# ViTAE-Transformer/SAMRS

Hardware: AMD Instinct MI355X
Metric: images/sec (1024^2, vit_h, 32 boxes/img) SAM box->mask (higher is better)
Workload: dtype f16

## Files before the change

### samrs_amd/csrc/decoder_kernels.hip

```cpp
#include "common.h"
#include "kernels.h"
#include "postprocess_value.h"

namespace {

constexpr float TWO_PI = 6.283185307179586f;

__device__ __forceinline__ float pe_channel(const float* __restrict__ gauss, float cx01, float cy01, int ch, int half) {
    const int f = ch < half ? ch : ch - half;
    const float vx = 2.0f * cx01 - 1.0f, vy = 2.0f * cy01 - 1.0f;
    const float a = TWO_PI * (vx * gauss[f] + vy * gauss[half + f]);
    return ch < half ? sinf(a) : cosf(a);
}

__global__ void prompt_tokens_kernel(PromptParams p, float* __restrict__ tokens, float* __restrict__ tokens2, int T, int C) {
    const int j = blockIdx.x, b = blockIdx.y, ch = threadIdx.x;
    const int half = C / 2;
    const bool has_pts = p.point_coords != nullptr;
    const bool has_box = p.boxes != nullptr;
    const int npt = has_pts ? p.n_points + (has_box ? 0 : 1) : 0;
    float v;
    if (j == 0) {
        v = p.iou_token[ch];
    } else if (j < 5) {
// ... 235 lines not shown
            }
#pragma unroll
            for (int t = 0; t < T2I_TG; ++t) {
                float sc = 0.f;
#pragma unroll
                for (int c = 0; c < 8; ++c) sc += q[t][c] * kf[c];
                sc += __builtin_bit_cast(float, __builtin_amdgcn_update_dpp(0, __builtin_bit_cast(int, sc), 0xB1, 0xF, 0xF, true));
                sc = valid ? sc : T2I_NEG;
                const float mn = fmaxf(m[t], sc);
                const float corr = __builtin_amdgcn_exp2f(m[t] - mn);
                const float pj = valid ? __builtin_amdgcn_exp2f(sc - mn) : 0.f;
                l[t] = l[t] * corr + pj;
#pragma unroll
                for (int c = 0; c < 8; ++c) acc[t][c] = acc[t][c] * corr + pj * vf[c];
                m[t] = mn;
            }
        }
#pragma unroll
        for (int u = 0; u < U; ++u) { kk[u] = kn[u]; vv[u] = vn[u]; }
    }
#undef T2I_LOAD
#pragma unroll
    for (int off = 16; off <= 32; off <<= 1) {
#pragma unroll
        for (int t = 0; t < T2I_TG; ++t) {
            const float mo = __shfl_xor(m[t], off, 64), lo = __shfl_xor(l[t], off, 64);
            const float mn = fmaxf(m[t], mo);
            const float fs = __builtin_amdgcn_exp2f(m[t] - mn), fo = __builtin_amdgcn_exp2f(mo - mn);
            l[t] = l[t] * fs + lo * fo;
#pragma unroll
            for (int c = 0; c < 8; ++c) acc[t][c] = acc[t][c] * fs + __shfl_xor(acc[t][c], off, 64) * fo;
            m[t] = mn;
        }
    }
    if (lane < 16) {
#pragma unroll
        for (int t = 0; t < T2I_TG; ++t) {
            float* r = sm[wave][t][ch];
            r[0] = m[t]; r[1] = l[t];
#pragma unroll
            for (int c = 0; c < 8; ++c) r[2 + c] = acc[t][c];
        }
    }
    __syncthreads();
    if (threadIdx.x < T2I_TG * 16) {
        const int t = threadIdx.x >> 4, c16 = threadIdx.x & 15;
        float mm = sm[0][t][c16][0];
#pragma unroll
        for (int w = 1; w < 4; ++w) mm = fmaxf(mm, sm[w][t][c16][0]);
        float ll = 0.f, a[8] = {0.f, 0.f, 0.f, 0.f, 0.f, 0.f, 0.f, 0.f};
#pragma unroll
        for (int w = 0; w < 4; ++w) {
            const float f = __builtin_amdgcn_exp2f(sm[w][t][c16][0] - mm);
            ll += sm[w][t][c16][1] * f;
#pragma unroll
            for (int c = 0; c < 8; ++c) a[c] += sm[w][t][c16][2 + c] * f;
        }
        float* r = part + ((((size_t)b * gridDim.z + blockIdx.z) * gridDim.x + split) * (T2I_TG * 16) + threadIdx.x) * T2I_REC;
        r[0] = mm; r[1] = ll;
#pragma unroll
        for (int c = 0; c < 8; ++c) r[2 + c] = a[c];
    }
}

__global__ __launch_bounds__(T2I_TG * 16) void t2i_merge_kernel(const float* __restrict__ part, float* __restrict__ o,
                                                                int splits, int T, int Ci) {
    const int b = blockIdx.x, tg = blockIdx.y;
    const int t = tg * T2I_TG + (threadIdx.x >> 4), ch = threadIdx.x & 15;
    if (t >= T) return;
    const float* base = part + (((size_t)b * gridDim.y + tg) * splits * (T2I_TG * 16) + threadIdx.x) * T2I_REC;
    const size_t sstride = (size_t)(T2I_TG * 16) * T2I_REC;
    float mm = T2I_NEG;
    for (int s = 0; s < splits; ++s) mm = fmaxf(mm, base[s * sstride]);
    float ll = 0.f, a[8] = {0.f, 0.f, 0.f, 0.f, 0.f, 0.f, 0.f, 0.f};
    for (int s = 0; s < splits; ++s) {
        const float* r = base + s * sstride;
        const float f = __builtin_amdgcn_exp2f(r[0] - mm);
        ll += r[1] * f;
#pragma unroll
        for (int c = 0; c < 8; ++c) a[c] += r[2 + c] * f;
    }
    const float inv = 1.0f / ll;
    float* orow = o + ((size_t)b * T + t) * Ci + ch * 8;
#pragma unroll
    for (int c = 0; c < 8; ++c) orow[c] = a[c] * inv;
}

constexpr int I2T_HS = 20;
template <int PREC>
__global__ __launch_bounds__(256) void i2t_attention_kernel(const uint16_t* __restrict__ qi, int ld, long bstride,
                                                            const float* __restrict__ kt, const float* __restrict__ vt,
                                                            uint16_t* __restrict__ out, int T, int tokens, int Ci) {
    constexpr int HD = 16;
    extern __shared__ float sm[];
    const int heads = Ci / HD;
    const int RS = heads * I2T_HS;
    float* sk = sm;
    float* sv = sm + T * RS;
    const int b = blockIdx.y;
    for (int i = threadIdx.x; i < T * Ci; i += 256) {
        const int j = i / Ci, c = i % Ci;
        sk[j * RS + (c / HD) * I2T_HS + c % HD] = kt[(size_t)b * T * Ci + i];
        sv[j * RS + (c / HD) * I2T_HS + c % HD] = vt[(size_t)b * T * Ci + i];
    }
    __syncthreads();
    const int tok = blockIdx.x * (256 / heads) + threadIdx.x / heads;
    const int h = threadIdx.x % heads;
    if (tok >= tokens) return;
    const uint16_t* qrow = qi + ((size_t)b * bstride + tok) * ld + h * HD;
    const uint4 q0 = *reinterpret_cast<const uint4*>(qrow);
    const uint4 q1 = *reinterpret_cast<const uint4*>(qrow + 8);
    const uint32_t qw[8] = {q0.x, q0.y, q0.z, q0.w, q1.x, q1.y, q1.z, q1.w};
    float qf[HD];
#pragma unroll
    for (int c = 0; c < 8; ++c) {
        qf[2 * c] = ET<PREC>::to_float((uint16_t)(qw[c] & 0xffffu)) * 0.25f;
        qf[2 * c + 1] = ET<PREC>::to_float((uint16_t)(qw[c] >> 16)) * 0.25f;
    }
    float m = -INFINITY, l = 0.f, acc[HD];
#pragma unroll
    for (int c = 0; c < HD; ++c) acc[c] = 0.f;
    for (int j = 0; j < T; ++j) {
        float kr[HD], vr[HD];
#pragma unroll
        for (int c4 = 0; c4 < HD / 4; ++c4) {
            const float4 k4 = *reinterpret_cast<const float4*>(sk + j * RS + h * I2T_HS + 4 * c4);
            const float4 v4 = *reinterpret_cast<const float4*>(sv + j * RS + h * I2T_HS + 4 * c4);
            kr[4 * c4] = k4.x; kr[4 * c4 + 1] = k4.y; kr[4 * c4 + 2] = k4.z; kr[4 * c4 + 3] = k4.w;
            vr[4 * c4] = v4.x; vr[4 * c4 + 1] = v4.y; vr[4 * c4 + 2] = v4.z; vr[4 * c4 + 3] = v4.w;
        }
        float s = 0.f;
#pragma unroll
        for (int c = 0; c < HD; ++c) s += qf[c] * kr[c];
        const float mn = fmaxf(m, s);
        const float corr = __expf(m - mn), pj = __expf(s - mn);
        l = l * corr + pj;
#pragma unroll
        for (int c = 0; c < HD; ++c) acc[c] = acc[c] * corr + pj * vr[c];
        m = mn;
    }
    const float inv = 1.0f / l;
    uint4 o0, o1;
    o0.x = pack2<PREC>(acc[0] * inv, acc[1] * inv);   o0.y = pack2<PREC>(acc[2] * inv, acc[3] * inv);
    o0.z = pack2<PREC>(acc[4] * inv, acc[5] * inv);   o0.w = pack2<PREC>(acc[6] * inv, acc[7] * inv);
    o1.x = pack2<PREC>(acc[8] * inv, acc[9] * inv);   o1.y = pack2<PREC>(acc[10] * inv, acc[11] * inv);
    o1.z = pack2<PREC>(acc[12] * inv, acc[13] * inv); o1.w = pack2<PREC>(acc[14] * inv, acc[15] * inv);
    uint16_t* orow = out + ((size_t)b * tokens + tok) * Ci + h * HD;
    *reinterpret_cast<uint4*>(orow) = o0;
    *reinterpret_cast<uint4*>(orow + 8) = o1;
}

constexpr int I2TF_ROWS = 32;
constexpr int I2TF_AST = 136;

template <int PREC, bool SPLIT>
__global__ __launch_bounds__(256, 2) void i2t_fused_kernel(const uint16_t* __restrict__ qi, int ld, long q_bstride,
                                                        const int* __restrict__ slot_of, const float* __restrict__ kt, const float* __restrict__ vt,
                                                        const uint16_t* __restrict__ w, const uint16_t* __restrict__ w_lo,
                                                        const float* __restrict__ bias,
                                                        const float* __restrict__ resid, long r_bstride,
                                                        const float* __restrict__ gamma, const float* __restrict__ beta, float eps,
                                                        float* __restrict__ outF, uint16_t* __restrict__ outE,
                                                        uint16_t* __restrict__ outE_lo, int T, int tokens, int groups_per_block) {
    constexpr int HD = 16, HEADS = 8, CI = 128, CO = 256, NWV = 4;
    constexpr int KRS = HEADS * I2T_HS;
    extern __shared__ __attribute__((aligned(16))) unsigned char smraw[];
    float* sk = reinterpret_cast<float*>(smraw);
    float* sv = sk + T * KRS;
    float* sp = sv + T * KRS;
    float* ex = sp + 3 * CO;
    uint16_t* At = reinterpret_cast<uint16_t*>(ex + 2 * NWV * I2TF_ROWS);
    uint16_t* Al = At + I2TF_ROWS * I2TF_AST;
    const int tid = threadIdx.x, lane = tid & 63, wave = tid >> 6;
    const int fr = lane & 15, fq = lane >> 4;
    const int b = blockIdx.y;
    for (int i = tid; i < T * CI; i += 256) {
        const int j = i / CI, c = i % CI;
        sk[j * KRS + (c / HD) * I2T_HS + c % HD] = kt[(size_t)b * T * CI + i];
        sv[j * KRS + (c / HD) * I2T_HS + c % HD] = vt[(size_t)b * T * CI + i];
    }
    for (int i = tid; i < CO; i += 256) { sp[i] = bias[i]; sp[CO + i] = gamma[i]; sp[2 * CO + i] = beta[i]; }
    uint4 wf[4][4], wl[SPLIT ? 4 : 1][4];
#pragma unroll
    for (int i = 0; i < 4; ++i)
#pragma unroll
        for (int ks = 0; ks < 4; ++ks) {
            const size_t o = (size_t)(wave * 64 + i * 16 + fr) * CI + ks * 32 + fq * 8;
            wf[i][ks] = *reinterpret_cast<const uint4*>(w + o);
            if constexpr (SPLIT) wl[i][ks] = *reinterpret_cast<const uint4*>(w_lo + o);
        }
    __syncthreads();

    const int tr = tid >> 3, h = tid & 7;
    const int g0 = blockIdx.x * groups_per_block;
    const int ib = slot_of ? slot_of[b] : b;
    const uint16_t* qbase = qi + (size_t)ib * q_bstride * ld + (size_t)tr * ld + h * HD;
    uint4 q0 = make_uint4(0u, 0u, 0u, 0u), q1 = q0;
    if (g0 * I2TF_ROWS < tokens) {
        q0 = *reinterpret_cast<const uint4*>(qbase + (size_t)g0 * I2TF_ROWS * ld);
        q1 = *reinterpret_cast<const uint4*>(qbase + (size_t)g0 * I2TF_ROWS * ld + 8);
    }
    for (int g = g0; g < g0 + groups_per_block; ++g) {
        const int row0 = g * I2TF_ROWS;
        if (row0 >= tokens) break;
        float4 rs[2][4];
#pragma unroll
        for (int mt = 0; mt < 2; ++mt)
#pragma unroll
            for (int i = 0; i < 4; ++i)
                rs[mt][i] = *reinterpret_cast<const float4*>(resid + ((size_t)ib * r_bstride + row0 + mt * 16 + fr) * CO + wave * 64 + i * 16 + 4 * fq);
        {
            const uint32_t qw[8] = {q0.x, q0.y, q0.z, q0.w, q1.x, q1.y, q1.z, q1.w};
            float qf[HD];
#pragma unroll
            for (int c = 0; c < 8; ++c) {
                qf[2 * c] = ET<PREC>::to_float((uint16_t)(qw[c] & 0xffffu)) * 0.25f;
                qf[2 * c + 1] = ET<PREC>::to_float((uint16_t)(qw[c] >> 16)) * 0.25f;
            }
            float m = -INFINITY, l = 0.f, acc[HD];
#pragma unroll
            for (int c = 0; c < HD; ++c) acc[c] = 0.f;
            for (int j = 0; j < T; ++j) {
                float kr[HD], vr[HD];
#pragma unroll
                for (int c4 = 0; c4 < HD / 4; ++c4) {
                    const float4 k4 = *reinterpret_cast<const float4*>(sk + j * KRS + h * I2T_HS + 4 * c4);
                    const float4 v4 = *reinterpret_cast<const float4*>(sv + j * KRS + h * I2T_HS + 4 * c4);
                    kr[4 * c4] = k4.x; kr[4 * c4 + 1] = k4.y; kr[4 * c4 + 2] = k4.z; kr[4 * c4 + 3] = k4.w;
                    vr[4 * c4] = v4.x; vr[4 * c4 + 1] = v4.y; vr[4 * c4 + 2] = v4.z; vr[4 * c4 + 3] = v4.w;
                }
                float sc = 0.f;
#pragma unroll
                for (int c = 0; c < HD; ++c) sc += qf[c] * kr[c];
                const float mn = fmaxf(m, sc);
                const float corr = __expf(m - mn), pj = __expf(sc - mn);
                l = l * corr + pj;
#pragma unroll
                for (int c = 0; c < HD; ++c) acc[c] = acc[c] * corr + pj * vr[c];
                m = mn;
            }
            const float inv = 1.0f / l;
            uint32_t oh[8], ol[8];
#pragma unroll
            for (int c = 0; c < 8; ++c) split2_pack<PREC>(acc[2 * c] * inv, acc[2 * c + 1] * inv, oh[c], ol[c]);
            *reinterpret_cast<uint4*>(At + tr * I2TF_AST + h * HD) = make_uint4(oh[0], oh[1], oh[2], oh[3]);
            *reinterpret_cast<uint4*>(At + tr * I2TF_AST + h * HD + 8) = make_uint4(oh[4], oh[5], oh[6], oh[7]);
            if constexpr (SPLIT) {
                *reinterpret_cast<uint4*>(Al + tr * I2TF_AST + h * HD) = make_uint4(ol[0], ol[1], ol[2], ol[3]);
                *reinterpret_cast<uint4*>(Al + tr * I2TF_AST + h * HD + 8) = make_uint4(ol[4], ol[5], ol[6], ol[7]);
            }
        }
        __syncthreads();
        if (g + 1 < g0 + groups_per_block && (g + 1) * I2TF_ROWS < tokens) {
            q0 = *reinterpret_cast<const uint4*>(qbase + (size_t)(g + 1) * I2TF_ROWS * ld);
            q1 = *reinterpret_cast<const uint4*>(qbase + (size_t)(g + 1) * I2TF_ROWS * ld + 8);
        }
        float v[2][4][4];
        float s1[2];
#pragma unroll
        for (int mt = 0; mt < 2; ++mt) {
            uint4 af[4], al[SPLIT ? 4 : 1];
#pragma unroll
            for (int ks = 0; ks < 4; ++ks) {
                af[ks] = *reinterpret_cast<const uint4*>(At + (mt * 16 + fr) * I2TF_AST + ks * 32 + fq * 8);
                if constexpr (SPLIT) al[ks] = *reinterpret_cast<const uint4*>(Al + (mt * 16 + fr) * I2TF_AST + ks * 32 + fq * 8);
            }
            s1[mt] = 0.f;
#pragma unroll
            for (int i = 0; i < 4; ++i) {
                f32x4_t a = {0.f, 0.f, 0.f, 0.f};
                if constexpr (SPLIT) {
                    f32x4_t c = {0.f, 0.f, 0.f, 0.f};
#pragma unroll
                    for (int ks = 0; ks < 4; ++ks) c = ET<PREC>::mfma16(wf[i][ks], al[ks], c);
#pragma unroll
                    for (int ks = 0; ks < 4; ++ks) c = ET<PREC>::mfma16(wl[i][ks], af[ks], c);
                    a = c;
                }
#pragma unroll
                for (int ks = 0; ks < 4; ++ks) a = ET<PREC>::mfma16(wf[i][ks], af[ks], a);
                const float4 bb = *reinterpret_cast<const float4*>(sp + wave * 64 + i * 16 + 4 * fq);
                v[mt][i][0] = (a[0] + bb.x) + rs[mt][i].x; v[mt][i][1] = (a[1] + bb.y) + rs[mt][i].y;
                v[mt][i][2] = (a[2] + bb.z) + rs[mt][i].z; v[mt][i][3] = (a[3] + bb.w) + rs[mt][i].w;
                s1[mt] += (v[mt][i][0] + v[mt][i][1]) + (v[mt][i][2] + v[mt][i][3]);
            }
        }
#pragma unroll
        for (int mt = 0; mt < 2; ++mt) {
            s1[mt] += __shfl_xor(s1[mt], 16, 64);
            s1[mt] += __shfl_xor(s1[mt], 32, 64);
            if (fq == 0) ex[wave * I2TF_ROWS + mt * 16 + fr] = s1[mt];
        }
        __syncthreads();
        float mean[2], s2[2];
#pragma unroll
        for (int mt = 0; mt < 2; ++mt) {
            const int r = mt * 16 + fr;
            mean[mt] = ((ex[r] + ex[I2TF_ROWS + r]) + (ex[2 * I2TF_ROWS + r] + ex[3 * I2TF_ROWS + r])) * (1.0f / CO);
            s2[mt] = 0.f;
#pragma unroll
            for (int i = 0; i < 4; ++i)
#pragma unroll
                for (int r4 = 0; r4 < 4; ++r4) { v[mt][i][r4] -= mean[mt]; s2[mt] += v[mt][i][r4] * v[mt][i][r4]; }
            s2[mt] += __shfl_xor(s2[mt], 16, 64);
            s2[mt] += __shfl_xor(s2[mt], 32, 64);
            if (fq == 0) ex[NWV * I2TF_ROWS + wave * I2TF_ROWS + r] = s2[mt];
        }
        __syncthreads();
#pragma unroll
        for (int mt = 0; mt < 2; ++mt) {
            const int r = mt * 16 + fr;
            const float* e2 = ex + NWV * I2TF_ROWS;
            const float rstd = 1.0f / sqrtf(((e2[r] + e2[I2TF_ROWS + r]) + (e2[2 * I2TF_ROWS + r] + e2[3 * I2TF_ROWS + r])) * (1.0f / CO) + eps);
            const size_t orow = (size_t)b * tokens + row0 + r;
#pragma unroll
            for (int i = 0; i < 4; ++i) {
                const int n = wave * 64 + i * 16 + 4 * fq;
                const float4 gm = *reinterpret_cast<const float4*>(sp + CO + n), bt = *reinterpret_cast<const float4*>(sp + 2 * CO + n);
                const float y0 = v[mt][i][0] * rstd * gm.x + bt.x, y1 = v[mt][i][1] * rstd * gm.y + bt.y;
                const float y2 = v[mt][i][2] * rstd * gm.z + bt.z, y3 = v[mt][i][3] * rstd * gm.w + bt.w;
                if (outF) *reinterpret_cast<float4*>(outF + orow * CO + n) = make_float4(y0, y1, y2, y3);
                uint2 o, lo;
                split2_pack<PREC>(y0, y1, o.x, lo.x);
                split2_pack<PREC>(y2, y3, o.y, lo.y);
                *reinterpret_cast<uint2*>(outE + orow * CO + n) = o;
                if (outE_lo) *reinterpret_cast<uint2*>(outE_lo + orow * CO + n) = lo;
            }
        }
    }
}

template <int PREC>
__global__ __launch_bounds__(256) void group_ln_gelu_kernel(const float* __restrict__ in, const float* __restrict__ gamma,
                                                            const float* __restrict__ beta, float eps,
                                                            uint16_t* __restrict__ out, long rows) {
    const int lane = threadIdx.x & 63;
    const long row = (long)blockIdx.x * 4 + (threadIdx.x >> 6);
    if (row >= rows) return;
    const float4 v = reinterpret_cast<const float4*>(in + row * 256)[lane];
    float s = (v.x + v.y) + (v.z + v.w);
#pragma unroll
    for (int off = 8; off > 0; off >>= 1) s += __shfl_xor(s, off, 64);
    const float mean = s * (1.0f / 64.0f);
    const float a = v.x - mean, b = v.y - mean, c = v.z - mean, d = v.w - mean;
    float q = (a * a + b * b) + (c * c + d * d);
#pragma unroll
    for (int off = 8; off > 0; off >>= 1) q += __shfl_xor(q, off, 64);
    const float rstd = 1.0f / sqrtf(q * (1.0f / 64.0f) + eps);
    const int c0 = (lane & 15) * 4;
    const float4 g = *reinterpret_cast<const float4*>(gamma + c0);
    const float4 bt = *reinterpret_cast<const float4*>(beta + c0);
    uint2 o;
    const float2_t g0 = gelu_erf2(float2_t{a * rstd * g.x + bt.x, b * rstd * g.y + bt.y});
    const float2_t g1 = gelu_erf2(float2_t{c * rstd * g.z + bt.z, d * rstd * g.w + bt.w});
    o.x = pack2<PREC>(g0.x, g0.y);
    o.y = pack2<PREC>(g1.x, g1.y);
    reinterpret_cast<uint2*>(out + row * 256)[lane] = o;
}

template <int PREC>
__global__ __launch_bounds__(256) void mask_product_kernel(const uint16_t* __restrict__ up2, const float* __restrict__ hyper,
                                                           float* __restrict__ low, int grid, int n_mask_tokens,
                                                           int sel0, int n_sel) {
    __shared__ float hy[4][32];
    const int b = blockIdx.y;
    if (threadIdx.x < n_sel * 32)
        hy[threadIdx.x / 32][threadIdx.x % 32] = hyper[((size_t)b * n_mask_tokens + sel0 + threadIdx.x / 32) * 32 + threadIdx.x % 32];
    __syncthreads();
    const int S = 4 * grid;
    const int pix = blockIdx.x * 256 + threadIdx.x;
    const int Y = pix / S, X = pix % S;
    const int y = Y >> 2, dy = (Y >> 1) & 1, dy2 = Y & 1;
    const int x = X >> 2, dx = (X >> 1) & 1, dx2 = X & 1;
    const size_t prow = (((size_t)b * grid * grid + (size_t)y * grid + x) * 4 + dy * 2 + dx) * 4 + dy2 * 2 + dx2;
    const uint4* src = reinterpret_cast<const uint4*>(up2 + prow * 32);
    float u[32];
#pragma unroll
    for (int i = 0; i < 4; ++i) {
        const uint4 w = src[i];
        const uint32_t ww[4] = {w.x, w.y, w.z, w.w};
#pragma unroll
        for (int e = 0; e < 4; ++e) {
            u[i * 8 + 2 * e] = ET<PREC>::to_float((uint16_t)(ww[e] & 0xffffu));
            u[i * 8 + 2 * e + 1] = ET<PREC>::to_float((uint16_t)(ww[e] >> 16));
        }
    }
    for (int c = 0; c < n_sel; ++c) {
        float s = 0.f;
#pragma unroll
        for (int k = 0; k < 32; ++k) s += hy[c][k] * u[k];
        low[(((size_t)b * n_sel + c) * S + Y) * S + X] = s;
    }
}

constexpr int U2_GROUPS_PER_WAVE = 16;

template <int PREC, int NSEL, bool SPLIT>
__global__ __launch_bounds__(256) void upscale2_mask_kernel(const void* __restrict__ u1v, const uint16_t* __restrict__ w,
                                                            const uint16_t* __restrict__ w_lo,
                                                            const float* __restrict__ bias, const float* __restrict__ hyper,
                                                            float* __restrict__ low, int grid, int n_mask_tokens, int sel0) {
    const int lane = threadIdx.x & 63, wave = threadIdx.x >> 6;
    const int fr = lane & 15, fq = lane >> 4;
    const int b = blockIdx.y;
    const int rows_per_prompt = grid * grid * 4;
    const int S = 4 * grid;
    uint4 wf[8][2], wl[SPLIT ? 8 : 1][2];
    float bv[8][4], hy[NSEL][8];
#pragma unroll
    for (int i = 0; i < 8; ++i) {
#pragma unroll
        for (int ks = 0; ks < 2; ++ks) {
            wf[i][ks] = *reinterpret_cast<const uint4*>(w + (i * 16 + fr) * 64 + ks * 32 + fq * 8);
            if constexpr (SPLIT) wl[i][ks] = *reinterpret_cast<const uint4*>(w_lo + (i * 16 + fr) * 64 + ks * 32 + fq * 8);
        }
        const float4 t = *reinterpret_cast<const float4*>(bias + i * 16 + 4 * fq);
        bv[i][0] = t.x; bv[i][1] = t.y; bv[i][2] = t.z; bv[i][3] = t.w;
    }
#pragma unroll
    for (int c = 0; c < NSEL; ++c) {
        const float* h = hyper + ((size_t)b * n_mask_tokens + sel0 + c) * 32;
#pragma unroll
        for (int half = 0; half < 2; ++half) {
            const float4 t = *reinterpret_cast<const float4*>(h + half * 16 + 4 * fq);
            hy[c][half * 4 + 0] = t.x; hy[c][half * 4 + 1] = t.y; hy[c][half * 4 + 2] = t.z; hy[c][half * 4 + 3] = t.w;
        }
    }
    const int row0 = (blockIdx.x * 4 + wave) * (16 * U2_GROUPS_PER_WAVE);
    const uint16_t* abase = reinterpret_cast<const uint16_t*>(u1v) + ((size_t)b * rows_per_prompt + row0 + fr) * 64 + fq * 8;
    const float* fbase = reinterpret_cast<const float*>(u1v) + ((size_t)b * rows_per_prompt + row0 + fr) * 64 + fq * 8;
    uint4 a0 = make_uint4(0u, 0u, 0u, 0u), a1 = a0;
    float4 f[SPLIT ? 4 : 1];
    if constexpr (SPLIT) {
        f[0] = *reinterpret_cast<const float4*>(fbase); f[1] = *reinterpret_cast<const float4*>(fbase + 4);
        f[2] = *reinterpret_cast<const float4*>(fbase + 32); f[3] = *reinterpret_cast<const float4*>(fbase + 36);
    } else {
        a0 = *reinterpret_cast<const uint4*>(abase); a1 = *reinterpret_cast<const uint4*>(abase + 32);
    }
    for (int g = 0; g < U2_GROUPS_PER_WAVE; ++g) {
        uint4 c0 = a0, c1 = a1, l0 = make_uint4(0u, 0u, 0u, 0u), l1 = l0;
        if constexpr (SPLIT) {
            split2_pack<PREC>(f[0].x, f[0].y, c0.x, l0.x); split2_pack<PREC>(f[0].z, f[0].w, c0.y, l0.y);
            split2_pack<PREC>(f[1].x, f[1].y, c0.z, l0.z); split2_pack<PREC>(f[1].z, f[1].w, c0.w, l0.w);
            split2_pack<PREC>(f[2].x, f[2].y, c1.x, l1.x); split2_pack<PREC>(f[2].z, f[2].w, c1.y, l1.y);
            split2_pack<PREC>(f[3].x, f[3].y, c1.z, l1.z); split2_pack<PREC>(f[3].z, f[3].w, c1.w, l1.w);
        }
        if (g + 1 < U2_GROUPS_PER_WAVE) {
            if constexpr (SPLIT) {
                const float* nb = fbase + (size_t)(g + 1) * 16 * 64;
                f[0] = *reinterpret_cast<const float4*>(nb); f[1] = *reinterpret_cast<const float4*>(nb + 4);
                f[2] = *reinterpret_cast<const float4*>(nb + 32); f[3] = *reinterpret_cast<const float4*>(nb + 36);
            } else {
                a0 = *reinterpret_cast<const uint4*>(abase + (size_t)(g + 1) * 16 * 64);
                a1 = *reinterpret_cast<const uint4*>(abase + (size_t)(g + 1) * 16 * 64 + 32);
            }
        }
        float part[NSEL][4];
#pragma unroll
        for (int c = 0; c < NSEL; ++c)
#pragma unroll
            for (int q = 0; q < 4; ++q) part[c][q] = 0.f;
#pragma unroll
        for (int i = 0; i < 8; ++i) {
            f32x4_t acc = {0.f, 0.f, 0.f, 0.f};
            if constexpr (SPLIT) {
                acc = ET<PREC>::mfma16(wf[i][0], l0, acc);
                acc = ET<PREC>::mfma16(wf[i][1], l1, acc);
                acc = ET<PREC>::mfma16(wl[i][0], c0, acc);
                acc = ET<PREC>::mfma16(wl[i][1], c1, acc);
            }
            acc = ET<PREC>::mfma16(wf[i][0], c0, acc);
            acc = ET<PREC>::mfma16(wf[i][1], c1, acc);
            const float2_t g01 = gelu_erf2(float2_t{acc[0] + bv[i][0], acc[1] + bv[i][1]});
            const float2_t g23 = gelu_erf2(float2_t{acc[2] + bv[i][2], acc[3] + bv[i][3]});
#pragma unroll
            for (int c = 0; c < NSEL; ++c) {
                const float* h = hy[c] + (i & 1) * 4;
                part[c][i >> 1] += h[0] * g01.x + h[1] * g01.y + h[2] * g23.x + h[3] * g23.y;
            }
// ... 314 lines not shown
    if (s >= n_in - 1) { f = 0.f; s = n_in - 1; }
    RTap t;
    t.i0 = s;
    t.i1 = s + 1 < n_in ? s + 1 : n_in - 1;
    t.w0 = 1.0f - f;
    t.w1 = f;
    return t;
}

__global__ __launch_bounds__(256) void rbox_prompt_kernel(const int32_t* __restrict__ pts, int nv, int h, int w, int th, int tw,
                                                          int img_size, int out_size, float* __restrict__ out, int fill_rule) {
#pragma clang fp contract(off)
    __shared__ RboxPoly P;
    const int b = blockIdx.y;
    if (threadIdx.x == 0) {
        P.nv = nv;
        P.rule = fill_rule;
        for (int e = 0; e < nv; ++e) { P.x[e] = pts[((size_t)b * nv + e) * 2]; P.y[e] = pts[((size_t)b * nv + e) * 2 + 1]; }
        for (int e = 0; e < nv; ++e) {
            const int a = e == 0 ? nv - 1 : e - 1;
            const long long x0 = P.x[a], y0 = P.y[a], x1 = P.x[e], y1 = P.y[e];
            if (y0 == y1) { P.ey0[e] = P.ey1[e] = 0; P.ex[e] = P.edx[e] = 0; continue; }
            P.edx[e] = ((x1 - x0) << 16) / (y1 - y0);
            if (y0 < y1) { P.ey0[e] = (int)y0; P.ey1[e] = (int)y1; P.ex[e] = x0 << 16; }
            else { P.ey0[e] = (int)y1; P.ey1[e] = (int)y0; P.ex[e] = x1 << 16; }
        }
    }
    __syncthreads();
    const int pix = blockIdx.x * 256 + threadIdx.x;
    if (pix >= out_size * out_size) return;
    const int oy = pix / out_size, ox = pix % out_size;
    const RTap by = rbox_tap(oy, img_size, out_size), bx = rbox_tap(ox, img_size, out_size);
    const int Ys[2] = {by.i0, by.i1}, Xs[2] = {bx.i0, bx.i1};
    double pv[2][2];
    for (int a = 0; a < 2; ++a)
        for (int c = 0; c < 2; ++c) {
            const int Y = Ys[a], X = Xs[c];
            if (Y >= th || X >= tw) { pv[a][c] = -1000.0; continue; }
            const RTap ay = rbox_tap(Y, h, th), ax = rbox_tap(X, w, tw);
            const double m00 = rbox_inside(P, ax.i0, ay.i0) ? 1000.0 : -1000.0;
            const double m01 = rbox_inside(P, ax.i1, ay.i0) ? 1000.0 : -1000.0;
            const double m10 = rbox_inside(P, ax.i0, ay.i1) ? 1000.0 : -1000.0;
            const double m11 = rbox_inside(P, ax.i1, ay.i1) ? 1000.0 : -1000.0;
            const double r0 = m00 * (double)ax.w0 + m01 * (double)ax.w1;
            const double r1 = m10 * (double)ax.w0 + m11 * (double)ax.w1;
            pv[a][c] = r0 * (double)ay.w0 + r1 * (double)ay.w1;
        }
    const double t0 = pv[0][0] * (double)bx.w0 + pv[0][1] * (double)bx.w1;
    const double t1 = pv[1][0] * (double)bx.w0 + pv[1][1] * (double)bx.w1;
    out[(size_t)b * out_size * out_size + pix] = (float)(t0 * (double)by.w0 + t1 * (double)by.w1);
}

}

hipError_t launch_resample_pass(const uint8_t* in, uint8_t* out, const int32_t* bounds, const int32_t* coef, int ksize,
                                int in_len, int out_len, int other, int horizontal, hipStream_t s) {
    const long total = (long)out_len * other * 3;
    resample_pass_kernel<<<(int)((total + 255) / 256), 256, 0, s>>>(in, out, bounds, coef, ksize, in_len, out_len, other, horizontal);
    return hipGetLastError();
}

hipError_t launch_prompt_tokens(const PromptParams& p, float* tokens, float* tokens2, int T, hipStream_t s) {
    dim3 g(T, p.n_prompts), b(256);
    prompt_tokens_kernel<<<g, b, 0, s>>>(p, tokens, tokens2, T, 256);
    return hipGetLastError();
}
hipError_t launch_dense_pe(const float* gauss, float* pe, int grid, hipStream_t s) {
    dense_pe_kernel<<<grid * grid, 256, 0, s>>>(gauss, pe, grid, 256);
    return hipGetLastError();
}
hipError_t launch_mask_embed(const MaskEmbedParams& p, const float* mask_in, float* dense, int n, int grid, hipStream_t s) {
    dim3 g(grid * grid / 16, n);
    mask_embed_kernel<<<g, 256, 0, s>>>(p, mask_in, dense, grid);
    return hipGetLastError();
}
hipError_t launch_fill_slot_table(const int* start, const int* slot, int n_runs, int* out, hipStream_t s) {
    for (int k0 = 0; k0 < n_runs; k0 += SLOT_RUNS_MAX) {
        SlotRuns r{};
        const int nr = n_runs - k0 < SLOT_RUNS_MAX ? n_runs - k0 : SLOT_RUNS_MAX;
        for (int k = 0; k < nr; ++k) { r.start[k] = start[k0 + k]; r.slot[k] = slot[k0 + k]; }
        r.start[nr] = start[k0 + nr];
        fill_slot_table_kernel<<<nr, 64, 0, s>>>(r, out);
    }
    return hipGetLastError();
}
hipError_t launch_make_keys(int prec, const float* emb, const float* dense, const float* vec, float* out_f32,
                            void* out_et, int n_batches, int tokens, int C, hipStream_t s, const int* slot_of) {
    const long per4 = (long)tokens * C / 4, tot4 = per4 * n_batches;
    const int blocks = (int)((tot4 + 255) / 256);
    if (prec == PREC_BF16)
        make_keys_kernel<PREC_BF16><<<blocks, 256, 0, s>>>(emb, slot_of, dense, vec, out_f32, (uint16_t*)out_et, per4, tot4, C / 4);
    else
        make_keys_kernel<PREC_F16><<<blocks, 256, 0, s>>>(emb, slot_of, dense, vec, out_f32, (uint16_t*)out_et, per4, tot4, C / 4);
    return hipGetLastError();
}
hipError_t launch_add_f32(const float* a, const float* b, float* out, long n, hipStream_t s) {
    if (n % 4) return hipErrorInvalidValue;
    add_f32_kernel<<<(int)((n / 4 + 255) / 256), 256, 0, s>>>(a, b, out, n / 4);
    return hipGetLastError();
}
hipError_t launch_token_self_attn(const float* q, const float* k, const float* v, float* o, int n, int T, int C,
                                  int heads, hipStream_t s) {
    if (C / heads != 32 || T > TOK_MAX) return hipErrorInvalidValue;
    token_self_attn_kernel<32><<<n, 256, 3 * T * C * sizeof(float), s>>>(q, k, v, o, T, C, heads);
    return hipGetLastError();
}
size_t t2i_workspace_floats(int n, int T) {
    return (size_t)n * ((T + T2I_TG - 1) / T2I_TG) * T2I_MAX_SPLITS * (T2I_TG * 16) * T2I_REC;
}
hipError_t launch_t2i_attention(int prec, const float* qp, const void* kp, const void* vp, int ld, long bstride,
                                float* o, float* workspace, int n, int T, int tokens, int Ci, int heads, hipStream_t s,
                                const int* slot_of) {
    if (Ci != 128 || heads != 8 || T > TOK_MAX || !workspace) return hipErrorInvalidValue;
    int splits = (tokens + 255) / 256;
    splits = splits < 1 ? 1 : (splits > T2I_MAX_SPLITS ? T2I_MAX_SPLITS : splits);
    const int kpw = ((tokens + splits * 4 - 1) / (splits * 4) + 15) / 16 * 16;
    const int tgs = (T + T2I_TG - 1) / T2I_TG;
    dim3 g(splits, n, tgs), b(256);
    const uint16_t* k = (const uint16_t*)kp;
    const uint16_t* v = (const uint16_t*)vp;
    if (prec == PREC_BF16) t2i_partial_kernel<PREC_BF16><<<g, b, 0, s>>>(qp, k, v, ld, bstride, slot_of, workspace, T, tokens, Ci, kpw);
    else t2i_partial_kernel<PREC_F16><<<g, b, 0, s>>>(qp, k, v, ld, bstride, slot_of, workspace, T, tokens, Ci, kpw);
    t2i_merge_kernel<<<dim3(n, tgs), T2I_TG * 16, 0, s>>>(workspace, o, splits, T, Ci);
    return hipGetLastError();
}
hipError_t launch_i2t_attention(int prec, const void* qi, int ld, long bstride, const float* kt, const float* vt,
                                void* out, int n, int T, int tokens, int Ci, int heads, hipStream_t s) {
    if (Ci / heads != 16 || 256 % heads) return hipErrorInvalidValue;
    const int per = 256 / heads;
    dim3 g((tokens + per - 1) / per, n), b(256);
    const size_t sh = 2 * (size_t)T * heads * I2T_HS * sizeof(float);
    if (prec == PREC_BF16)
        i2t_attention_kernel<PREC_BF16><<<g, b, sh, s>>>((const uint16_t*)qi, ld, bstride, kt, vt, (uint16_t*)out, T, tokens, Ci);
    else
        i2t_attention_kernel<PREC_F16><<<g, b, sh, s>>>((const uint16_t*)qi, ld, bstride, kt, vt, (uint16_t*)out, T, tokens, Ci);
    return hipGetLastError();
}
hipError_t launch_i2t_fused(int prec, const void* qi, int ld, long q_bstride, const float* kt, const float* vt, const void* w,
                            const void* w_lo, const float* bias, const float* resid, long r_bstride, const float* gamma,
                            const float* beta, float eps, float* outF, void* outE, void* outE_lo, int n, int T, int tokens, int Ci,
                            int C, hipStream_t s, const int* slot_of) {
    if (Ci != 128 || C != 256 || T < 1 || T > TOK_MAX || tokens % I2TF_ROWS) return hipErrorInvalidValue;
    const int groups = tokens / I2TF_ROWS;
    int gpb = 4;
    while (gpb > 1 && groups % gpb) gpb >>= 1;
    dim3 g(groups / gpb, n), b(256);
    const bool split = w_lo != nullptr;
    const size_t sh = (size_t)(2 * T * 8 * I2T_HS + 3 * 256 + 2 * 4 * I2TF_ROWS) * sizeof(float) +
                      (size_t)(split ? 2 : 1) * I2TF_ROWS * I2TF_AST * 2;
#define I2TF_LAUNCH(P, S)                                                                                                       \
    i2t_fused_kernel<P, S><<<g, b, sh, s>>>((const uint16_t*)qi, ld, q_bstride, slot_of, kt, vt, (const uint16_t*)w, (const uint16_t*)w_lo, \
                                           bias, resid, r_bstride, gamma, beta, eps, outF, (uint16_t*)outE, (uint16_t*)outE_lo, T, \
                                           tokens, gpb)
    if (prec == PREC_BF16) { if (split) I2TF_LAUNCH(PREC_BF16, true); else I2TF_LAUNCH(PREC_BF16, false); }
    else { if (split) I2TF_LAUNCH(PREC_F16, true); else I2TF_LAUNCH(PREC_F16, false); }
#undef I2TF_LAUNCH
    return hipGetLastError();
}
hipError_t launch_group_ln_gelu(int prec, const float* in, const float* gamma, const float* beta, float eps,
                                void* out, long rows, int groups, int gsize, hipStream_t s) {
    if (groups != 4 || gsize != 64) return hipErrorInvalidValue;
    const int blocks = (int)((rows + 3) / 4);
    if (prec == PREC_BF16) group_ln_gelu_kernel<PREC_BF16><<<blocks, 256, 0, s>>>(in, gamma, beta, eps, (uint16_t*)out, rows);
    else group_ln_gelu_kernel<PREC_F16><<<blocks, 256, 0, s>>>(in, gamma, beta, eps, (uint16_t*)out, rows);
    return hipGetLastError();
}
hipError_t launch_mask_product(int prec, const void* up2, const float* hyper, float* low, int n, int grid,
                               int n_mask_tokens, int sel0, int n_sel, hipStream_t s) {
    if (n_sel > 4 || n_sel < 1) return hipErrorInvalidValue;
    const int S = 4 * grid;
    dim3 g(S * S / 256, n), b(256);
    if (prec == PREC_BF16) mask_product_kernel<PREC_BF16><<<g, b, 0, s>>>((const uint16_t*)up2, hyper, low, grid, n_mask_tokens, sel0, n_sel);
    else mask_product_kernel<PREC_F16><<<g, b, 0, s>>>((const uint16_t*)up2, hyper, low, grid, n_mask_tokens, sel0, n_sel);
    return hipGetLastError();
}
hipError_t launch_upscale2_masks(int prec, const void* u1, const void* w, const void* w_lo, const float* bias, const float* hyper,
                                 float* low, int n, int grid, int n_mask_tokens, int sel0, int n_sel, hipStream_t s) {
    const int rows_per_block = 4 * 16 * U2_GROUPS_PER_WAVE;
    if ((grid * grid * 4) % rows_per_block || (n_sel != 1 && n_sel != 3)) return hipErrorInvalidValue;
    dim3 g(grid * grid * 4 / rows_per_block, n), b(256);
    const uint16_t* ww = (const uint16_t*)w;
    const uint16_t* wl = (const uint16_t*)w_lo;
#define U2_LAUNCH(P, NS, SP) upscale2_mask_kernel<P, NS, SP><<<g, b, 0, s>>>(u1, ww, wl, bias, hyper, low, grid, n_mask_tokens, sel0)
#define U2_SEL(P, SP) do { if (n_sel == 1) U2_LAUNCH(P, 1, SP); else U2_LAUNCH(P, 3, SP); } while (0)
    if (prec == PREC_BF16) { if (w_lo) U2_SEL(PREC_BF16, true); else U2_SEL(PREC_BF16, false); }
    else { if (w_lo) U2_SEL(PREC_F16, true); else U2_SEL(PREC_F16, false); }
#undef U2_SEL
#undef U2_LAUNCH
    return hipGetLastError();
}
hipError_t launch_postprocess(const float* low, int n_masks, int in_h, int in_w, int orig_h, int orig_w,
                              int img_size, int return_logits, void* out, hipStream_t s) {
    const long work = (long)((orig_w + 3) / 4) * orig_h;
    dim3 g((unsigned)((work + 255) / 256), n_masks), b(256);
    postprocess_kernel<<<g, b, 0, s>>>(low, img_size / 4, in_h, in_w, orig_h, orig_w, img_size, return_logits, out);
    return hipGetLastError();
}
hipError_t launch_paint(const uint8_t* masks, const int32_t* labels, int n, int h, int w, uint8_t* seg,
                        unsigned long long* areas, unsigned long long* class_pixels,
                        unsigned long long* class_instances, int n_classes, hipStream_t s) {
    const long hw = (long)h * w;
    const bool fused = seg && areas && hw % 16 == 0 && (((uintptr_t)masks | (uintptr_t)seg) & 15) == 0;
    if (seg && !fused) paint_kernel<<<(int)((hw + 255) / 256), 256, 0, s>>>(masks, labels, n, hw, seg);
    if (areas) {
        HIP_CHECK_RET(hipMemsetAsync(areas, 0, sizeof(unsigned long long) * n, s));
        if (fused) {
            paint_area_kernel<<<(int)((hw / 16 + 255) / 256), 256, 0, s>>>(masks, labels, n, hw, seg, areas);
        } else {
            dim3 g(64, n);
            area_kernel<<<g, 256, 0, s>>>(masks, hw, areas);
        }
        if (class_pixels || class_instances)
            class_stats_kernel<<<1, 64, 0, s>>>(areas, labels, n, class_pixels, class_instances, n_classes);
    }
    return hipGetLastError();
}

hipError_t launch_select_best(const uint8_t* masks, const float* iou, int n, int nsel, int h, int w, uint8_t* out, float* quality,
                              unsigned long long* areas, hipStream_t s) {
    if (n < 1 || nsel < 1 || h < 1 || w < 1) return hipErrorInvalidValue;
    const long hw = (long)h * w;
    HIP_CHECK_RET(hipMemsetAsync(areas, 0, sizeof(unsigned long long) * n, s));
    int chunks = (int)((hw / 16 + 255) / 256);
    chunks = chunks < 1 ? 1 : (chunks > 64 ? 64 : chunks);
    select_best_kernel<<<dim3(chunks, n), 256, 0, s>>>(masks, iou, nsel, hw, out, quality, areas);
    return hipGetLastError();
}

hipError_t launch_gt_match(const uint8_t* masks, int n, int h, int w, const uint8_t* label_rgb, const uint8_t* colors,
                           unsigned long long* inter, unsigned long long* gt_area, uint8_t* gt_masks, hipStream_t s) {
    const long hw = (long)h * w;
    if (n < 1 || h < 1 || w < 1 || hw >= (1l << 30)) return hipErrorInvalidValue;
    HIP_CHECK_RET(hipMemsetAsync(inter, 0, sizeof(unsigned long long) * n, s));
    HIP_CHECK_RET(hipMemsetAsync(gt_area, 0, sizeof(unsigned long long) * n, s));
    const int blocks = (int)(((hw + 15) / 16 + 255) / 256);
    gt_match_kernel<<<blocks, 256, 0, s>>>(masks, n, hw, label_rgb, colors, inter, gt_area, gt_masks);
    return hipGetLastError();
}

hipError_t launch_rbox_prompt(const int32_t* pts, int n, int nv, int h, int w, int th, int tw, int img_size, int out_size,
                              float* out, hipStream_t s, int fill_rule) {
    if (n < 1 || nv < 3 || nv > RBOX_MAXV || h < 1 || w < 1 || th < 1 || tw < 1 || th > img_size || tw > img_size || out_size < 1 ||
        fill_rule < 0 || fill_rule > 1)
        return hipErrorInvalidValue;
    dim3 g((out_size * out_size + 255) / 256, n), b(256);
    rbox_prompt_kernel<<<g, b, 0, s>>>(pts, nv, h, w, th, tw, img_size, out_size, out, fill_rule);
    return hipGetLastError();
}
```

Baseline: 148.7.

## Warp-specialize image-to-token fused kernel with double-buffered attention/projection pipeline

Adds a 512-thread variant of the image-to-token fused kernel. Four producer waves compute the per-row attention into a double-buffered LDS tile while four consumer waves run the MFMA output projection, residual add and LayerNorm on the previous tile. The consumer waves keep their weight fragments in registers for the whole block. Each block now processes more row groups, chosen from the launch size. It is enabled by default and can be turned off with an env var. In exchange it uses more LDS and registers per block and adds barriers, which may lower occupancy.

```diff
diff --git a/samrs_amd/csrc/decoder_kernels.hip b/samrs_amd/csrc/decoder_kernels.hip
--- a/samrs_amd/csrc/decoder_kernels.hip
+++ b/samrs_amd/csrc/decoder_kernels.hip
@@ -411,6 +411,51 @@
 
 constexpr int I2TF_ROWS = 32;
 constexpr int I2TF_AST = 136;
+
+template <int PREC, bool SPLIT>
+__device__ __forceinline__ void i2tf_attend(const uint4 q0, const uint4 q1, const float* sk, const float* sv, int T, int h,
+                                            uint16_t* at, uint16_t* al) {
+    constexpr int HD = 16, KRS = 8 * I2T_HS;
+    const uint32_t qw[8] = {q0.x, q0.y, q0.z, q0.w, q1.x, q1.y, q1.z, q1.w};
+    float qf[HD];
+#pragma unroll
+    for (int c = 0; c < 8; ++c) {
+        qf[2 * c] = ET<PREC>::to_float((uint16_t)(qw[c] & 0xffffu)) * 0.25f;
+        qf[2 * c + 1] = ET<PREC>::to_float((uint16_t)(qw[c] >> 16)) * 0.25f;
+    }
+    float m = -INFINITY, l = 0.f, acc[HD];
+#pragma unroll
+    for (int c = 0; c < HD; ++c) acc[c] = 0.f;
+    for (int j = 0; j < T; ++j) {
+        float kr[HD], vr[HD];
+#pragma unroll
+        for (int c4 = 0; c4 < HD / 4; ++c4) {
+            const float4 k4 = *reinterpret_cast<const float4*>(sk + j * KRS + h * I2T_HS + 4 * c4);
+            const float4 v4 = *reinterpret_cast<const float4*>(sv + j * KRS + h * I2T_HS + 4 * c4);
+            kr[4 * c4] = k4.x; kr[4 * c4 + 1] = k4.y; kr[4 * c4 + 2] = k4.z; kr[4 * c4 + 3] = k4.w;
+            vr[4 * c4] = v4.x; vr[4 * c4 + 1] = v4.y; vr[4 * c4 + 2] = v4.z; vr[4 * c4 + 3] = v4.w;
+        }
+        float sc = 0.f;
+#pragma unroll
+        for (int c = 0; c < HD; ++c) sc += qf[c] * kr[c];
+        const float mn = fmaxf(m, sc);
+        const float corr = __expf(m - mn), pj = __expf(sc - mn);
+        l = l * corr + pj;
+#pragma unroll
+        for (int c = 0; c < HD; ++c) acc[c] = acc[c] * corr + pj * vr[c];
+        m = mn;
+    }
+    const float inv = 1.0f / l;
+    uint32_t oh[8], ol[8];
+#pragma unroll
+    for (int c = 0; c < 8; ++c) split2_pack<PREC>(acc[2 * c] * inv, acc[2 * c + 1] * inv, oh[c], ol[c]);
+    *reinterpret_cast<uint4*>(at) = make_uint4(oh[0], oh[1], oh[2], oh[3]);
+    *reinterpret_cast<uint4*>(at + 8) = make_uint4(oh[4], oh[5], oh[6], oh[7]);
+    if constexpr (SPLIT) {
+        *reinterpret_cast<uint4*>(al) = make_uint4(ol[0], ol[1], ol[2], ol[3]);
+        *reinterpret_cast<uint4*>(al + 8) = make_uint4(ol[4], ol[5], ol[6], ol[7]);
+    }
+}
 
 template <int PREC, bool SPLIT>
 __global__ __launch_bounds__(256, 2) void i2t_fused_kernel(const uint16_t* __restrict__ qi, int ld, long q_bstride,
@@ -468,47 +513,7 @@
 #pragma unroll
             for (int i = 0; i < 4; ++i)
                 rs[mt][i] = *reinterpret_cast<const float4*>(resid + ((size_t)ib * r_bstride + row0 + mt * 16 + fr) * CO + wave * 64 + i * 16 + 4 * fq);
-        {
-            const uint32_t qw[8] = {q0.x, q0.y, q0.z, q0.w, q1.x, q1.y, q1.z, q1.w};
-            float qf[HD];
-#pragma unroll
-            for (int c = 0; c < 8; ++c) {
-                qf[2 * c] = ET<PREC>::to_float((uint16_t)(qw[c] & 0xffffu)) * 0.25f;
-                qf[2 * c + 1] = ET<PREC>::to_float((uint16_t)(qw[c] >> 16)) * 0.25f;
-            }
-            float m = -INFINITY, l = 0.f, acc[HD];
-#pragma unroll
-            for (int c = 0; c < HD; ++c) acc[c] = 0.f;
-            for (int j = 0; j < T; ++j) {
-                float kr[HD], vr[HD];
-#pragma unroll
-                for (int c4 = 0; c4 < HD / 4; ++c4) {
-                    const float4 k4 = *reinterpret_cast<const float4*>(sk + j * KRS + h * I2T_HS + 4 * c4);
-                    const float4 v4 = *reinterpret_cast<const float4*>(sv + j * KRS + h * I2T_HS + 4 * c4);
-                    kr[4 * c4] = k4.x; kr[4 * c4 + 1] = k4.y; kr[4 * c4 + 2] = k4.z; kr[4 * c4 + 3] = k4.w;
-                    vr[4 * c4] = v4.x; vr[4 * c4 + 1] = v4.y; vr[4 * c4 + 2] = v4.z; vr[4 * c4 + 3] = v4.w;
-                }
-                float sc = 0.f;
-#pragma unroll
-                for (int c = 0; c < HD; ++c) sc += qf[c] * kr[c];
-                const float mn = fmaxf(m, sc);
-                const float corr = __expf(m - mn), pj = __expf(sc - mn);
-                l = l * corr + pj;
-#pragma unroll
-                for (int c = 0; c < HD; ++c) acc[c] = acc[c] * corr + pj * vr[c];
-                m = mn;
-            }
-            const float inv = 1.0f / l;
-            uint32_t oh[8], ol[8];
-#pragma unroll
-            for (int c = 0; c < 8; ++c) split2_pack<PREC>(acc[2 * c] * inv, acc[2 * c + 1] * inv, oh[c], ol[c]);
-            *reinterpret_cast<uint4*>(At + tr * I2TF_AST + h * HD) = make_uint4(oh[0], oh[1], oh[2], oh[3]);
-            *reinterpret_cast<uint4*>(At + tr * I2TF_AST + h * HD + 8) = make_uint4(oh[4], oh[5], oh[6], oh[7]);
-            if constexpr (SPLIT) {
-                *reinterpret_cast<uint4*>(Al + tr * I2TF_AST + h * HD) = make_uint4(ol[0], ol[1], ol[2], ol[3]);
-                *reinterpret_cast<uint4*>(Al + tr * I2TF_AST + h * HD + 8) = make_uint4(ol[4], ol[5], ol[6], ol[7]);
-            }
-        }
+        i2tf_attend<PREC, SPLIT>(q0, q1, sk, sv, T, h, At + tr * I2TF_AST + h * HD, Al + tr * I2TF_AST + h * HD);
         __syncthreads();
         if (g + 1 < g0 + groups_per_block && (g + 1) * I2TF_ROWS < tokens) {
             q0 = *reinterpret_cast<const uint4*>(qbase + (size_t)(g + 1) * I2TF_ROWS * ld);
@@ -584,6 +589,163 @@
                 split2_pack<PREC>(y2, y3, o.y, lo.y);
                 *reinterpret_cast<uint2*>(outE + orow * CO + n) = o;
                 if (outE_lo) *reinterpret_cast<uint2*>(outE_lo + orow * CO + n) = lo;
+            }
+        }
+    }
+}
+
+template <int PREC, bool SPLIT>
+__global__ __launch_bounds__(512, 2) void i2t_fused_pipe_kernel(const uint16_t* __restrict__ qi, int ld, long q_bstride,
+                                                             const int* __restrict__ slot_of, const float* __restrict__ kt, const float* __restrict__ vt,
+                                                             const uint16_t* __restrict__ w, const uint16_t* __restrict__ w_lo,
+                                                             const float* __restrict__ bias,
+                                                             const float* __restrict__ resid, long r_bstride,
+                                                             const float* __restrict__ gamma, const float* __restrict__ beta, float eps,
+                                                             float* __restrict__ outF, uint16_t* __restrict__ outE,
+                                                             uint16_t* __restrict__ outE_lo, int T, int tokens, int groups_per_block) {
+    constexpr int HD = 16, HEADS = 8, CI = 128, CO = 256, NWV = 4;
+    constexpr int KRS = HEADS * I2T_HS;
+    constexpr int ATILE = I2TF_ROWS * I2TF_AST, ABUF = (SPLIT ? 2 : 1) * ATILE;
+    extern __shared__ __attribute__((aligned(16))) unsigned char smraw[];
+    float* sk = reinterpret_cast<float*>(smraw);
+    float* sv = sk + T * KRS;
+    float* sp = sv + T * KRS;
+    float* ex = sp + 3 * CO;
+    uint16_t* A0 = reinterpret_cast<uint16_t*>(ex + 2 * NWV * I2TF_ROWS);
+    const int tid = threadIdx.x, lane = tid & 63, wave = tid >> 6;
+    const int b = blockIdx.y;
+    for (int i = tid; i < T * CI; i += 512) {
+        const int j = i / CI, c = i % CI;
+        sk[j * KRS + (c / HD) * I2T_HS + c % HD] = kt[(size_t)b * T * CI + i];
+        sv[j * KRS + (c / HD) * I2T_HS + c % HD] = vt[(size_t)b * T * CI + i];
+    }
+    for (int i = tid; i < CO; i += 512) { sp[i] = bias[i]; sp[CO + i] = gamma[i]; sp[2 * CO + i] = beta[i]; }
+    const int g0 = blockIdx.x * groups_per_block;
+    const int ng = min(groups_per_block, tokens / I2TF_ROWS - g0);
+    const int ib = slot_of ? slot_of[b] : b;
+
+    if (wave >= NWV) {
+        const int pt = tid - NWV * 64, tr = pt >> 3, h = pt & 7;
+        const uint16_t* qbase = qi + (size_t)ib * q_bstride * ld + ((size_t)g0 * I2TF_ROWS + tr) * ld + h * HD;
+        uint16_t* at = A0 + tr * I2TF_AST + h * HD;
+        uint4 q0 = *reinterpret_cast<const uint4*>(qbase), q1 = *reinterpret_cast<const uint4*>(qbase + 8);
+        __syncthreads();
+        for (int k = 0; k <= ng; ++k) {
+            if (k < ng) {
+                uint4 n0 = q0, n1 = q1;
+                if (k + 1 < ng) {
+                    n0 = *reinterpret_cast<const uint4*>(qbase + (size_t)(k + 1) * I2TF_ROWS * ld);
+                    n1 = *reinterpret_cast<const uint4*>(qbase + (size_t)(k + 1) * I2TF_ROWS * ld + 8);
+                }
+                i2tf_attend<PREC, SPLIT>(q0, q1, sk, sv, T, h, at + (k & 1) * ABUF, at + (k & 1) * ABUF + ATILE);
+                q0 = n0; q1 = n1;
+            }
+            if (k > 0) __syncthreads();
+            __syncthreads();
+        }
+        return;
+    }
+
+    const int fr = lane & 15, fq = lane >> 4;
+    uint4 wf[4][4], wl[SPLIT ? 4 : 1][4];
+#pragma unroll
+    for (int i = 0; i < 4; ++i)
+#pragma unroll
+        for (int ks = 0; ks < 4; ++ks) {
+            const size_t o = (size_t)(wave * 64 + i * 16 + fr) * CI + ks * 32 + fq * 8;
+            wf[i][ks] = *reinterpret_cast<const uint4*>(w + o);
+            if constexpr (SPLIT) wl[i][ks] = *reinterpret_cast<const uint4*>(w_lo + o);
+        }
+    const float* rblk = resid + ((size_t)ib * r_bstride + (size_t)g0 * I2TF_ROWS) * CO;
+    const size_t oblk = ((size_t)b * tokens + (size_t)g0 * I2TF_ROWS) * CO;
+    const unsigned toff = fr * CO + wave * 64 + 4 * fq;
+    float4 rs[2][4];
+#pragma unroll
+    for (int mt = 0; mt < 2; ++mt)
+#pragma unroll
+        for (int i = 0; i < 4; ++i) rs[mt][i] = *reinterpret_cast<const float4*>(rblk + (toff + mt * 16 * CO + i * 16));
+    __syncthreads();
+    __syncthreads();
+    for (int k = 0; k < ng; ++k) {
+        const uint16_t* At = A0 + (k & 1) * ABUF;
+        const uint16_t* Al = At + ATILE;
+        float v[2][4][4];
+        float s1[2];
+#pragma unroll
+        for (int mt = 0; mt < 2; ++mt) {
+            uint4 af[4], al[SPLIT ? 4 : 1];
+#pragma unroll
+            for (int ks = 0; ks < 4; ++ks) {
+                af[ks] = *reinterpret_cast<const uint4*>(At + (mt * 16 + fr) * I2TF_AST + ks * 32 + fq * 8);
+                if constexpr (SPLIT) al[ks] = *reinterpret_cast<const uint4*>(Al + (mt * 16 + fr) * I2TF_AST + ks * 32 + fq * 8);
+            }
+            s1[mt] = 0.f;
+#pragma unroll
+            for (int i = 0; i < 4; ++i) {
+                f32x4_t a = {0.f, 0.f, 0.f, 0.f};
+                if constexpr (SPLIT) {
+                    f32x4_t c = {0.f, 0.f, 0.f, 0.f};
+#pragma unroll
+                    for (int ks = 0; ks < 4; ++ks) c = ET<PREC>::mfma16(wf[i][ks], al[ks], c);
+#pragma unroll
+                    for (int ks = 0; ks < 4; ++ks) c = ET<PREC>::mfma16(wl[i][ks], af[ks], c);
+                    a = c;
+                }
+#pragma unroll
+                for (int ks = 0; ks < 4; ++ks) a = ET<PREC>::mfma16(wf[i][ks], af[ks], a);
+                const float4 bb = *reinterpret_cast<const float4*>(sp + wave * 64 + i * 16 + 4 * fq);
+                v[mt][i][0] = (a[0] + bb.x) + rs[mt][i].x; v[mt][i][1] = (a[1] + bb.y) + rs[mt][i].y;
+                v[mt][i][2] = (a[2] + bb.z) + rs[mt][i].z; v[mt][i][3] = (a[3] + bb.w) + rs[mt][i].w;
+                s1[mt] += (v[mt][i][0] + v[mt][i][1]) + (v[mt][i][2] + v[mt][i][3]);
+            }
+        }
+        if (k + 1 < ng) {
+#pragma unroll
+            for (int mt = 0; mt < 2; ++mt)
+#pragma unroll
+                for (int i = 0; i < 4; ++i)
+                    rs[mt][i] = *reinterpret_cast<const float4*>(rblk + (toff + ((k + 1) * I2TF_ROWS + mt * 16) * CO + i * 16));
+        }
+#pragma unroll
+        for (int mt = 0; mt < 2; ++mt) {
+            s1[mt] += __shfl_xor(s1[mt], 16, 64);
+            s1[mt] += __shfl_xor(s1[mt], 32, 64);
+            if (fq == 0) ex[wave * I2TF_ROWS + mt * 16 + fr] = s1[mt];
+        }
+        __syncthreads();
+        float mean[2], s2[2];
+#pragma unroll
+        for (int mt = 0; mt < 2; ++mt) {
+            const int r = mt * 16 + fr;
+            mean[mt] = ((ex[r] + ex[I2TF_ROWS + r]) + (ex[2 * I2TF_ROWS + r] + ex[3 * I2TF_ROWS + r])) * (1.0f / CO);
+            s2[mt] = 0.f;
+#pragma unroll
+            for (int i = 0; i < 4; ++i)
+#pragma unroll
+                for (int r4 = 0; r4 < 4; ++r4) { v[mt][i][r4] -= mean[mt]; s2[mt] += v[mt][i][r4] * v[mt][i][r4]; }
+            s2[mt] += __shfl_xor(s2[mt], 16, 64);
+            s2[mt] += __shfl_xor(s2[mt], 32, 64);
+            if (fq == 0) ex[NWV * I2TF_ROWS + wave * I2TF_ROWS + r] = s2[mt];
+        }
+        __syncthreads();
+#pragma unroll
+        for (int mt = 0; mt < 2; ++mt) {
+            const int r = mt * 16 + fr;
+            const float* e2 = ex + NWV * I2TF_ROWS;
+            const float rstd = 1.0f / sqrtf(((e2[r] + e2[I2TF_ROWS + r]) + (e2[2 * I2TF_ROWS + r] + e2[3 * I2TF_ROWS + r])) * (1.0f / CO) + eps);
+            const unsigned orow = toff + (k * I2TF_ROWS + mt * 16) * CO;
+#pragma unroll
+            for (int i = 0; i < 4; ++i) {
+                const int n = wave * 64 + i * 16 + 4 * fq;
+                const float4 gm = *reinterpret_cast<const float4*>(sp + CO + n), bt = *reinterpret_cast<const float4*>(sp + 2 * CO + n);
+                const float y0 = v[mt][i][0] * rstd * gm.x + bt.x, y1 = v[mt][i][1] * rstd * gm.y + bt.y;
+                const float y2 = v[mt][i][2] * rstd * gm.z + bt.z, y3 = v[mt][i][3] * rstd * gm.w + bt.w;
+                if (outF) *reinterpret_cast<float4*>(outF + oblk + (orow + i * 16)) = make_float4(y0, y1, y2, y3);
+                uint2 o, lo;
+                split2_pack<PREC>(y0, y1, o.x, lo.x);
+                split2_pack<PREC>(y2, y3, o.y, lo.y);
+                *reinterpret_cast<uint2*>(outE + oblk + (orow + i * 16)) = o;
+                if (outE_lo) *reinterpret_cast<uint2*>(outE_lo + oblk + (orow + i * 16)) = lo;
             }
         }
     }
@@ -1204,6 +1366,21 @@
     i2t_fused_kernel<P, S><<<g, b, sh, s>>>((const uint16_t*)qi, ld, q_bstride, slot_of, kt, vt, (const uint16_t*)w, (const uint16_t*)w_lo, \
                                            bias, resid, r_bstride, gamma, beta, eps, outF, (uint16_t*)outE, (uint16_t*)outE_lo, T, \
                                            tokens, gpb)
+    static const bool pipe = [] { const char* v = getenv("SAMRS_I2T_PIPE"); return !(v && atoi(v) == 0); }();
+    if (pipe) {
+        int pg = 32;
+        while (pg > 4 && (long)n * ((groups + pg - 1) / pg) < 4 * 256) pg >>= 1;
+        const dim3 gp((groups + pg - 1) / pg, n), bp(512);
+        const size_t shp = sh + (size_t)(split ? 2 : 1) * I2TF_ROWS * I2TF_AST * 2;
+#define I2TF_PIPE_LAUNCH(P, S)                                                                                                  \
+    i2t_fused_pipe_kernel<P, S><<<gp, bp, shp, s>>>((const uint16_t*)qi, ld, q_bstride, slot_of, kt, vt, (const uint16_t*)w,     \
+                                                     (const uint16_t*)w_lo, bias, resid, r_bstride, gamma, beta, eps, outF,     \
+                                                     (uint16_t*)outE, (uint16_t*)outE_lo, T, tokens, pg)
+        if (prec == PREC_BF16) { if (split) I2TF_PIPE_LAUNCH(PREC_BF16, true); else I2TF_PIPE_LAUNCH(PREC_BF16, false); }
+        else { if (split) I2TF_PIPE_LAUNCH(PREC_F16, true); else I2TF_PIPE_LAUNCH(PREC_F16, false); }
+#undef I2TF_PIPE_LAUNCH
+        return hipGetLastError();
+    }
     if (prec == PREC_BF16) { if (split) I2TF_LAUNCH(PREC_BF16, true); else I2TF_LAUNCH(PREC_BF16, false); }
     else { if (split) I2TF_LAUNCH(PREC_F16, true); else I2TF_LAUNCH(PREC_F16, false); }
 #undef I2TF_LAUNCH
```

Measured after the change: 148.7, median of 3. About the same (-0.0%).
